# 924973292/EDITOR

Hardware: AMD Instinct MI355X
Metric: tri-modal images/sec fwd+bwd @ B=128 ViT-B (higher is better)
Workload: dtype bf16

## Files before the change

editor_amd/csrc/attention_bf16.hip:

```cpp
#include "common.h"
#include "../../include/editor_hip.h"
#include <type_traits>

#include "attn_common.h"
#include <string.h>

namespace {

#ifndef ATTN_ROLLOUT_SKIP
#define ATTN_ROLLOUT_SKIP 1
#endif
#ifndef ATTN_PAIR_SKIP
#define ATTN_PAIR_SKIP 0
#endif
#ifndef ATTN_UNROLL_BWD
#define ATTN_UNROLL_BWD 1
#endif

constexpr int STG_ROW = ROWB + 32, STG_BYTES = 16 * STG_ROW;
constexpr int STG_LPR = CPR <= 4 ? 4 : (CPR <= 8 ? 8 : 16);
template <bool F16>
__device__ __forceinline__ void store_tile(char* stg, const float4_t (&o)[ND], bf16_t* dst, long ldo, int nrows, int lane)
{
    const int li = lane & 15, lg = lane >> 4;
// ... 489 lines not shown
    if (kCols<NT> && a.colparts) {
        __syncthreads();
        float* red = reinterpret_cast<float*>(smem);
        wave_colsum_park(csk, red + (w * 2) * HD, lane);
        wave_colsum_park(csv, red + (w * 2 + 1) * HD, lane);
        __syncthreads();
        if (threadIdx.x < 2 * HD) {
            const int which = threadIdx.x / HD, c = threadIdx.x % HD;
            float t = 0.f;
            for (int i = 0; i < nw; ++i) t += red[(i * 2 + which) * HD + c];
            a.colparts[(long)b * 3 * D + (1 + which) * D + hh * HD + c] = t;
        }
    }
}

template <int NT, bool F16>
__global__ __launch_bounds__(256) __attribute__((amdgpu_waves_per_eu(4, 8))) void attn_rollout_step_kernel(const bf16_t* __restrict__ qkv, const float* __restrict__ lse,
    const float* __restrict__ r_in, int T, int heads, float scale, long Mtot, float* __restrict__ r_out, int final_step)
{
    extern __shared__ __attribute__((aligned(16))) char smem[];
    constexpr int Tp = NT * 16;
    char* qimg = smem;
    float* lse_s = reinterpret_cast<float*>(smem + Tp * ROWB);
    float* w_s = lse_s + Tp;
    const int D = heads * HD;
    const int b = blockIdx.x / heads, hh = blockIdx.x % heads;
    const long ld = 3L * D;
    const long row0 = (long)b * T;
    const int nt = min(NT, ((T + 31) >> 5) << 1);
    const int nu = !ATTN_ROLLOUT_SKIP ? nt : (r_in ? min(nt, (T + 15) >> 4) : 1);
// ... 7 lines not shown
    short8_t kn[KS];
#pragma unroll
    for (int s = 0; s < KS; ++s) kn[s] = frag_own(qbase + D, ld, w * 16, T, s, lane);
    images_ready();
    const int li = lane & 15, lg = lane >> 4;
    const float sc = scale * kLog2e;
    for (int k0 = w * 16; k0 < T; k0 += nw * 16) {
        const int key = k0 + li;
        short8_t kf[KS];
#pragma unroll
        for (int s = 0; s < KS; ++s) kf[s] = kn[s];
        if (k0 + nw * 16 < T) {
#pragma unroll
            for (int s = 0; s < KS; ++s) kn[s] = frag_own(qbase + D, ld, k0 + nw * 16, T, s, lane);
        }
        float acc = 0.f;
#pragma unroll 2
        for (int u = 0; u < nu; ++u) {
            float4_t s_ = {0.f, 0.f, 0.f, 0.f};
#pragma unroll
            for (int s = 0; s < KS; ++s)
                s_ = mfma16<F16>(frag_k(qimg, u * 16, s, lane), kf[s], s_);
            const float4 l4 = *reinterpret_cast<const float4*>(lse_s + 16 * u + 4 * lg);
            const float4 w4 = *reinterpret_cast<const float4*>(w_s + 16 * u + 4 * lg);
            acc = fmaf(__builtin_amdgcn_exp2f(s_[0] * sc - l4.x), w4.x, acc);
            acc = fmaf(__builtin_amdgcn_exp2f(s_[1] * sc - l4.y), w4.y, acc);
            acc = fmaf(__builtin_amdgcn_exp2f(s_[2] * sc - l4.z), w4.z, acc);
            acc = fmaf(__builtin_amdgcn_exp2f(s_[3] * sc - l4.w), w4.w, acc);
        }
        acc = group_sum(acc);
        if (lg == 0 && key < T) {
            if (final_step) { if (key >= 1) r_out[(long)blockIdx.x * (T - 1) + key - 1] = acc; }
            else r_out[(long)blockIdx.x * T + key] = acc;
        }
    }
}

constexpr int LCH = 256;

template <bool BWD, bool F16>
__global__ __launch_bounds__(256) __attribute__((amdgpu_waves_per_eu(4, 8))) void attn_q_long_kernel(AttnArgs a)
{
    extern __shared__ __attribute__((aligned(16))) char smem[];
    char* kimg = smem;
    char* vimg = smem + LCH * ROWB;
    const int D = a.heads * HD;
    const int b = blockIdx.x / a.heads, hh = blockIdx.x % a.heads;
    const long ld = 3L * D;
    const long row0 = a.cu ? (long)a.cu[b] : (long)b * a.T;
// ... 347 lines not shown
#define ROLL_CASE(NTV) case NTV: {                                                                                   \
        auto k = attn_rollout_step_kernel<NTV, F16>;                                                                     \
        const size_t lds = (size_t)NTV * 16 * ROWB + (size_t)2 * NTV * 16 * sizeof(float);                              \
        int rc = set_lds(k, lds); if (rc) return rc;                                                                     \
        hipLaunchKernelGGL(k, grid, dim3(threads), lds, stream, qkv, lse, r_in, T, heads, scale, Mtot, r_out, final_step); \
        break; }
    switch (pick_nt(T)) {
        ROLL_CASE(10) ROLL_CASE(14) ROLL_CASE(26) ROLL_CASE(38)
        default: return (int)hipErrorInvalidValue;
    }
#undef ROLL_CASE
    EDITOR_LAUNCH_CHECK();
    return 0;
}

}

#if ATTN_HD == 64
#define ATTN_ENTRY(name) name
#define ATTN_DECL_WIDTHS(name, ...) extern "C" int name##_hd32(__VA_ARGS__); extern "C" int name##_hd96(__VA_ARGS__);
#define ATTN_OTHER_WIDTHS(name, ...) do { if (hd == 32) return name##_hd32(__VA_ARGS__); if (hd == 96) return name##_hd96(__VA_ARGS__); } while (0)
#elif ATTN_HD == 32
#define ATTN_ENTRY(name) name##_hd32
#define ATTN_DECL_WIDTHS(name, ...)
#define ATTN_OTHER_WIDTHS(name, ...) do { } while (0)
#else
#define ATTN_ENTRY(name) name##_hd96
#define ATTN_DECL_WIDTHS(name, ...)
#define ATTN_OTHER_WIDTHS(name, ...) do { } while (0)
#endif
// ... 52 lines not shown
#define ROLL_ARGS const uint16_t* qkv, const float* lse, const float* r_in, int B, int T, int heads, int hd, float scale, \
                  float* r_out, int final_step, hipStream_t stream
ATTN_DECL_WIDTHS(editor_attn_rollout_step_bf16, ROLL_ARGS)
ATTN_DECL_WIDTHS(editor_attn_rollout_step_f16, ROLL_ARGS)
extern "C" int ATTN_ENTRY(editor_attn_rollout_step_bf16)(ROLL_ARGS)
{
    ATTN_OTHER_WIDTHS(editor_attn_rollout_step_bf16, qkv, lse, r_in, B, T, heads, hd, scale, r_out, final_step, stream);
    return rollout_step_h16<false>(qkv, lse, r_in, B, T, heads, hd, scale, r_out, final_step, stream);
}
extern "C" int ATTN_ENTRY(editor_attn_rollout_step_f16)(ROLL_ARGS)
{
    ATTN_OTHER_WIDTHS(editor_attn_rollout_step_f16, qkv, lse, r_in, B, T, heads, hd, scale, r_out, final_step, stream);
    return rollout_step_h16<true>(qkv, lse, r_in, B, T, heads, hd, scale, r_out, final_step, stream);
}
#undef ROLL_ARGS
```

editor_amd/csrc/gemm_f32.hip:

```cpp
#include "common.h"
#include "../../include/editor_hip.h"

typedef __attribute__((ext_vector_type(4))) float float4_t;

namespace {

constexpr int BM = 64, BN = 64, BK = 16, LDT = 80;

struct GemmArgs {
    const float* A; const float* B; float* C;
    int M, N, K;
    long lda, ldb, ldc;
    int transA, transB;
    int batch2; long sA1, sB1, sC1, sA2, sB2, sC2;
    float alpha, beta;
    const float* bias; const float* rowscale;
    int splitk;
    int epilogue; float* aux; long ldaux;
};

__device__ __forceinline__ float gelu_f(float a) { return 0.5f * a * (1.f + erff(a * 0.70710678118654752f)); }
__device__ __forceinline__ float gelu_grad_f(float a) {
    return 0.5f * (1.f + erff(a * 0.70710678118654752f)) + a * 0.3989422804014327f * __expf(-0.5f * a * a);
}

constexpr int NH = BK / 16;
struct TileRegs { float v[NH][4]; };

__device__ __forceinline__ void load_tile(const float* __restrict__ P, long ld, int trans, int r0, int k0, int R, int kend, TileRegs& t)
{
#pragma unroll
    for (int h = 0; h < NH; ++h) {
        const int c = threadIdx.x + 256 * h;
        float* v = t.v[h];
        v[0] = v[1] = v[2] = v[3] = 0.f;
        if (!trans) {
            const int r = c / (BK / 4), kk = (c % (BK / 4)) * 4;
            const int gr = r0 + r, gk = k0 + kk;
            if (gr < R) {
                const float* src = P + (long)gr * ld + gk;
                if (gk + 3 < kend && ((reinterpret_cast<uintptr_t>(src) & 15) == 0)) {
                    const float4 q = *reinterpret_cast<const float4*>(src);
                    v[0] = q.x; v[1] = q.y; v[2] = q.z; v[3] = q.w;
                } else {
#pragma unroll
                    for (int i = 0; i < 4; ++i) if (gk + i < kend) v[i] = src[i];
                }
            }
        } else {
            const int kk = c >> 4, r = (c & 15) * 4;
            const int gk = k0 + kk, gr = r0 + r;
            if (gk < kend) {
                const float* src = P + (long)gk * ld + gr;
                if (gr + 3 < R && ((reinterpret_cast<uintptr_t>(src) & 15) == 0)) {
                    const float4 q = *reinterpret_cast<const float4*>(src);
                    v[0] = q.x; v[1] = q.y; v[2] = q.z; v[3] = q.w;
                } else {
#pragma unroll
                    for (int i = 0; i < 4; ++i) if (gr + i < R) v[i] = src[i];
                }
            }
        }
    }
}
__device__ __forceinline__ void store_tile(const TileRegs& t, int trans, float (*S)[LDT])
{
#pragma unroll
    for (int h = 0; h < NH; ++h) {
        const int c = threadIdx.x + 256 * h;
        const float* v = t.v[h];
        if (!trans) {
            const int r = c / (BK / 4), kk = (c % (BK / 4)) * 4;
#pragma unroll
            for (int i = 0; i < 4; ++i) S[kk + i][r] = v[i];
        } else {
            const int kk = c >> 4, r = (c & 15) * 4;
            *reinterpret_cast<float4*>(&S[kk][r]) = make_float4(v[0], v[1], v[2], v[3]);
        }
    }
}

__global__ __launch_bounds__(256) __attribute__((amdgpu_waves_per_eu(4, 8))) void gemm_f32_kernel(GemmArgs g)
{
    __shared__ __attribute__((aligned(16))) float As[2][BK][LDT];
    __shared__ __attribute__((aligned(16))) float Bs[2][BK][LDT];
    const int z = blockIdx.z;
    const int split = z % g.splitk, bz = z / g.splitk;
    const int b1 = bz / g.batch2, b2 = bz % g.batch2;
    const float* A = g.A + b1 * g.sA1 + b2 * g.sA2;
    const float* B = g.B + b1 * g.sB1 + b2 * g.sB2;
    float* C = g.C + b1 * g.sC1 + b2 * g.sC2;
    const int m0 = blockIdx.y * BM, n0 = blockIdx.x * BN;
    const int ktiles = (g.K + BK - 1) / BK;
    const int per = (ktiles + g.splitk - 1) / g.splitk;
    const int kt0 = split * per, kt1 = min(ktiles, kt0 + per);
    const int lane = threadIdx.x & 63, w = threadIdx.x >> 6;
    const int wm = (w >> 1) * 32, wn = (w & 1) * 32;
    float4_t acc[2][2];
#pragma unroll
    for (int i = 0; i < 2; ++i)
#pragma unroll
        for (int j = 0; j < 2; ++j) acc[i][j] = float4_t{0.f, 0.f, 0.f, 0.f};

    TileRegs ra, rb;
    if (kt0 < kt1) {
        load_tile(A, g.lda, g.transA, m0, kt0 * BK, g.M, g.K, ra);
        load_tile(B, g.ldb, g.transB, n0, kt0 * BK, g.N, g.K, rb);
        store_tile(ra, g.transA, As[0]);
        store_tile(rb, g.transB, Bs[0]);
    }
    __syncthreads();
    for (int kt = kt0; kt < kt1; ++kt) {
        const int cur = (kt - kt0) & 1;
        const bool more = kt + 1 < kt1;
        if (more) {
            load_tile(A, g.lda, g.transA, m0, (kt + 1) * BK, g.M, g.K, ra);
            load_tile(B, g.ldb, g.transB, n0, (kt + 1) * BK, g.N, g.K, rb);
        }
#pragma unroll
        for (int ks = 0; ks < BK; ks += 4) {
            const int kr = ks + (lane >> 4);
            float a[2], b[2];
#pragma unroll
            for (int i = 0; i < 2; ++i) a[i] = As[cur][kr][wm + i * 16 + (lane & 15)];
#pragma unroll
            for (int j = 0; j < 2; ++j) b[j] = Bs[cur][kr][wn + j * 16 + (lane & 15)];
#pragma unroll
            for (int i = 0; i < 2; ++i)
#pragma unroll
                for (int j = 0; j < 2; ++j)
                    acc[i][j] = __builtin_amdgcn_mfma_f32_16x16x4f32(a[i], b[j], acc[i][j], 0, 0, 0);
        }
        if (more) {
            store_tile(ra, g.transA, As[cur ^ 1]);
            store_tile(rb, g.transB, Bs[cur ^ 1]);
        }
        __syncthreads();
    }
#pragma unroll
    for (int i = 0; i < 2; ++i)
#pragma unroll
        for (int j = 0; j < 2; ++j)
#pragma unroll
            for (int r = 0; r < 4; ++r) {
                const int m = m0 + wm + i * 16 + (lane >> 4) * 4 + r;
                const int n = n0 + wn + j * 16 + (lane & 15);
                if (m >= g.M || n >= g.N) continue;
                float v = g.alpha * acc[i][j][r];
                if (g.bias && split == 0) v += g.bias[n];
                if (g.rowscale) v *= g.rowscale[m];
                if (g.epilogue == EDITOR_EPI_RESIDUAL) v += g.aux[(long)m * g.ldaux + n];
                else if (g.epilogue == EDITOR_EPI_GELU) { g.aux[(long)m * g.ldaux + n] = v; v = gelu_f(v); }
                else if (g.epilogue == EDITOR_EPI_GELU_BWD) v *= gelu_grad_f(g.aux[(long)m * g.ldaux + n]);
                float* c = C + (long)m * g.ldc + n;
                if (g.splitk > 1) atomicAdd(c, v);
                else *c = g.beta != 0.f ? v + g.beta * *c : v;
            }
}

__global__ void scale_inplace_kernel(float* C, long rows, int cols, long ld, float beta)
{
    const long e = (long)blockIdx.x * blockDim.x + threadIdx.x;
    if (e >= rows * cols) return;
    float* c = C + (e / cols) * ld + (e % cols);
    *c = beta == 0.f ? 0.f : *c * beta;
}

}

extern "C" int editor_gemm_f32(const float* A, const float* B, float* C, int M, int N, int K, long lda, long ldb,
    long ldc, int transA, int transB, int batch1, long sA1, long sB1, long sC1, int batch2, long sA2, long sB2, long sC2,
    float alpha, float beta, const float* bias, const float* rowscale, int splitk, int epilogue, float* aux, long ldaux,
// ... 11 lines not shown
                float* c = C + b1 * sC1 + b2 * sC2;
                if (beta != 1.f) {
                    hipLaunchKernelGGL(scale_inplace_kernel, dim3((unsigned)(((long)M * N + 255) / 256)), dim3(256), 0,
                                       stream, c, (long)M, N, ldc, beta);
                    EDITOR_LAUNCH_CHECK();
                }
            }
    }
    GemmArgs g{A, B, C, M, N, K, lda, ldb, ldc, transA, transB, batch2, sA1, sB1, sC1, sA2, sB2, sC2,
               alpha, beta, bias, rowscale, splitk, epilogue, aux, ldaux};
    dim3 grid((N + BN - 1) / BN, (M + BM - 1) / BM, batch1 * batch2 * splitk);
    hipLaunchKernelGGL(gemm_f32_kernel, grid, dim3(256), 0, stream, g);
    EDITOR_LAUNCH_CHECK();
    return 0;
}
```

editor_amd/functional.py:

```python
import os
import weakref

import torch

from . import ops

_BF16_CACHE = {}
_WEIGHT_EPOCH = 0

F16_GRAD_SCALE = 32768.0


def set_f16_grad_scale(v):
    global F16_GRAD_SCALE
    v = float(v)
    if v <= 0 or (v != 2.0 ** round(__import__("math").log2(v))):
        raise ValueError("GRAD_SCALE must be a positive power of two")
    F16_GRAD_SCALE = v


def grad_scale(dtype):
    return F16_GRAD_SCALE if dtype == torch.float16 else 1.0


# ... 241 lines not shown



def _linear_bwd(*args, **kw):
    return _drive(_linear_bwd_gen(*args, **kw))


def _linear_bwd_gen(dy, x2d, w_act, need_bias, gelu_pre=None, m_live=None, db=None, dx_colsum=None, gs=1.0, dw_out=None,
                    db_out=None, dxcs_out=None, w_t=None, defer=None, aux_is_grad=True, rq=None, live_dense=False):
    m, n = dy.shape
    k = x2d.shape[1]
    inv = 1.0 / gs
    use_side = WGRAD_SIDE_STREAM and dy.dtype in ops.HALF_DTYPES and m >= 2048
    dy_ready = torch.cuda.current_stream(dy.device).record_event() if use_side else None
    dx = torch.empty(m, k, dtype=x2d.dtype, device=dy.device)
    dxcs = None
    if dx_colsum and ops.gemm_colsum_ok(m, k, n, dx.dtype, 0, 1, m_live, live_dense):
        dxcs = dxcs_out if dxcs_out is not None else torch.empty(k, dtype=torch.float32, device=dy.device)
    wb, ldb, tb = (w_t, n, 0) if w_t is not None else (w_act, k, 1)
    if gelu_pre is None:
        yield _GemmReq(dy, wb, dx, m, k, n, n, ldb, k, 0, tb, m_live=m_live, colsum=dxcs, colsum_scale=inv, tag="dgrad",
                       rq=rq, live_dense=live_dense)
    else:
        ag = ops.EPI_AUX_GRAD if (dy.dtype in ops.HALF_DTYPES and aux_is_grad) else 0
        yield _GemmReq(dy, wb, dx, m, k, n, n, ldb, k, 0, tb, epilogue=ops.EPI_GELU_BWD | ag | (STAGGER_FC2D if (m_live is None or live_dense) and m >= 16384 else 0),
                       aux=gelu_pre, m_live=m_live,
                       colsum=dxcs, colsum_scale=inv, tag="dgrad", rq=rq, live_dense=live_dense)
    dw = dw_out if dw_out is not None else torch.empty(n, k, dtype=torch.float32, device=dy.device)
    if need_bias and db is None:
        db = db_out if db_out is not None else torch.empty(n, dtype=torch.float32, device=dy.device)
# ... 619 lines not shown
```

editor_amd/ops.py:

```python
import ctypes
import os

import torch

from . import _lib

call = _lib.call
_raw_stream = _lib._raw_stream


def patch_grid(h, w, sy, sx=None):
    sx = sy if sx is None else sx
    return (h - 16) // sy + 1, (w - 16) // sx + 1


def freq_counts(rgb, nir, tir, m4=None, stride=16):
    b, c, h, w = rgb.shape
    if stride != 16:
        ny, nx = patch_grid(h, w, stride)
        counts = torch.empty(b, ny * nx, dtype=torch.int32, device=rgb.device)
        plane = torch.empty(b * h * (w // 16), dtype=torch.int16, device=rgb.device)
        if m4 is not None:
            call("editor_freq_counts_stride_nmod_f32", rgb.contiguous(), nir.contiguous(), tir.contiguous(), m4.contiguous(), 4,
                 b, c, h, w, int(stride), plane, counts)
# ... 23 lines not shown
    return mask


def frequency_mask(rgb, nir, tir, keep, m4=None, stride=16):
    counts = freq_counts(rgb, nir, tir, m4, stride)
    return topk_mask(counts, keep), counts


def attn_rollout(probs):
    l, b, h, t, ldp = probs.shape
    scores = torch.empty(b, h, t - 1, dtype=torch.float32, device=probs.device)
    call("editor_attn_rollout_f32", probs, l, b * h, t, ldp, b * h * t * ldp, scores)
    return scores


def attn_rollout_qk(layers, b, t, heads, hd, scale=None):
    dev = layers[0][0].device
    scores = torch.empty(b, heads, t - 1, dtype=torch.float32, device=dev)
    bufs = [torch.empty(b * heads, t, dtype=torch.float32, device=dev) for _ in range(2)]
    r_in = None
    for i, layer in enumerate(reversed(layers)):
        last = i == len(layers) - 1
        out = scores if last else bufs[i & 1]
        if len(layer) == 3:
            qkv, qkv_lo, lse = layer
            call("editor_attn_rollout_step_f16x2", qkv, qkv_lo, lse, r_in, b, t, heads, hd, float(scale or hd ** -0.5), out,
                 1 if last else 0)
        else:
            qkv, lse = layer
            call(_h16(qkv, "attn_rollout_step"), qkv, lse, r_in, b, t, heads, hd, float(scale or hd ** -0.5), out,
                 1 if last else 0)
        r_in = out
    return scores
# ... 6 lines not shown


_WS = {}
_WS_RETIRED = []


def workspace(device, nfloats):
    key = (device.type, device.index, _raw_stream(device.index if device.index is not None else torch.cuda.current_device()))
    ws = _WS.get(key)
    if ws is None or ws.numel() < nfloats:
        if ws is not None:
            _WS_RETIRED.append(ws)
        ws = torch.empty(max(int(nfloats), 1 << 22), dtype=torch.float32, device=device)
        _WS[key] = ws
    return ws


_ARENA = {}


class ReduceQueue:
    ARENA_FLOATS = 16 << 20

    def __init__(self, device, slot=0, nslots=1):
        key = (device.index, _raw_stream(device.index if device.index is not None else torch.cuda.current_device()))
        buf = _ARENA.get(key)
        if buf is None:
            buf = _ARENA[key] = torch.empty(self.ARENA_FLOATS, dtype=torch.float32, device=device)
        span = (self.ARENA_FLOATS // int(nslots)) // 64 * 64
        self.base, self.limit = int(slot) * span, (int(slot) + 1) * span
# ... 324 lines not shown

def gemm_tile_plan(m, n, cus=256):
    th = gemm_tile_rows(m, n, cus)
    tiles_pp = -(-m // th) * ((n + 255) // 256)
    tiles_pipe = -(-m // 256) * ((n + 127) // 128)
    cost_pp = -(-tiles_pp // cus) * (0.95 if th == 208 else 1.0)
    cost_pipe = -(-tiles_pipe // cus) * 0.69
    return th, cost_pipe < 0.97 * cost_pp


def gemm_colsum_ok(m, n, k, c_dtype, trans_a, splitk, m_live, live_dense=False):
    return (c_dtype in HALF_DTYPES and not trans_a and splitk == 1 and (m_live is None or live_dense) and m >= 2048 and n >= 512
            and n % 8 == 0 and k % 64 == 0)


def gemm(a, b, c, m, n, k, lda, ldb, ldc, trans_a=0, trans_b=0, alpha=1.0, beta=0.0, bias=None, rowscale=None,
         splitk=1, a_off=0, b_off=0, c_off=0, epilogue=0, aux=None, m_live=None, colsum=None, colsum_scale=1.0, tag=None,
         rq=None, live_dense=False, rowmap=None):
    if a.dtype == torch.float32:
        assert b.dtype == torch.float32 and c.dtype == torch.float32 and m_live is None
        if (splitk == 1 and not trans_a and not trans_b and m <= 512 and k >= 1024 and k % 128 == 0 and epilogue == 0
                and rowscale is None and beta == 0.0 and ldc == n and a_off == b_off == c_off == 0):
            s_ = 8
            kc = k // s_
            slabs = workspace(a.device, (s_ - 1) * m * n)
            call("editor_gemm_f32", a, b, c, m, n, kc, lda, ldb, ldc, 0, 0, 1, 0, 0, 0, 1, 0, 0, 0, float(alpha), 0.0, bias,
                 None, 1, 0, None, n)
            call("editor_gemm_f32", _ptr(a, kc), _ptr(b, kc), slabs, m, n, kc, lda, ldb, n, 0, 0, s_ - 1, kc, kc, m * n,
                 1, 0, 0, 0, float(alpha), 0.0, None, None, 1, 0, None, n)
            call("editor_reduce_rows", slabs, s_ - 1, m * n, c, 1, 1.0)
            return
        call("editor_gemm_f32", _ptr(a, a_off), _ptr(b, b_off), _ptr(c, c_off), m, n, k, lda, ldb, ldc,
             int(trans_a), int(trans_b), 1, 0, 0, 0, 1, 0, 0, 0, float(alpha), float(beta), bias, rowscale, int(splitk),
             int(epilogue) & 0xFF, aux, n)
    elif a.dtype in HALF_DTYPES:
        assert b.dtype == a.dtype
        entry = _h16(a, "gemm")
        if m_live is not None and (m < 256 or n < 128 or k % 64):
            raise RuntimeError("live-row GEMM needs the pipelined path (M >= 256, N >= 128, K % 64 == 0)")
# ... 538 lines not shown
```

include/editor_hip.h:

```cpp
#ifndef EDITOR_HIP_H
#define EDITOR_HIP_H
#include <stdint.h>
#ifdef __cplusplus
extern "C" {
#endif

typedef struct ihipStream_t* editor_stream_t;

#define EDITOR_EPI_NONE 0
#define EDITOR_EPI_RESIDUAL 1
#define EDITOR_EPI_GELU 2
#define EDITOR_EPI_GELU_BWD 3
#define EDITOR_EPI_COLSUM 0x100
#define EDITOR_EPI_AUX_GRAD 0x400
#define EDITOR_EPI_FORCE_PP 0x200
#define EDITOR_EPI_PIPE128 0x800
#define EDITOR_EPI_STAGGER(c) (((c) & 63) << 17)
#define EDITOR_EPI_TILE_ROWS(h) ((((h) / 16) & 15) << 12)


int editor_freq_counts_f32(const float* rgb, const float* nir, const float* tir, int B, int C, int H, int W,
                           int32_t* counts, editor_stream_t stream);

int editor_freq_counts_nmod_f32(const float* m0, const float* m1, const float* m2, const float* m3, int nmod, int B, int C,
// ... 83 lines not shown

int editor_sfts_apply(const float* feat, const uint8_t* index, int nmod, long B, int T, int D, float* out,
                      float* loss, float* workspace, int ws_len, editor_stream_t stream);
int editor_sfts_apply_bwd(const float* feat, const uint8_t* index, const float* dout, const float* dloss, int nmod,
                          long B, int T, int D, float* dfeat, editor_stream_t stream);
int editor_pool_fwd(const float* x, long B, int nmod, int T, int D, float* out, float* num, editor_stream_t stream);
int editor_pool_bwd(const float* dout, const float* num, long B, int nmod, int T, int D, float* dx,
                    editor_stream_t stream);
int editor_rowmask_mul(float* x, const uint8_t* rowmask, int period, long M, int D, editor_stream_t stream);


int editor_gemm_f32(const float* A, const float* B, float* C, int M, int N, int K, long lda, long ldb, long ldc,
                    int transA, int transB, int batch1, long sA1, long sB1, long sC1, int batch2, long sA2, long sB2,
                    long sC2, float alpha, float beta, const float* bias, const float* rowscale, int splitk,
                    int epilogue, float* aux, long ldaux, editor_stream_t stream);

int editor_gemm_bf16(const uint16_t* A, const uint16_t* B, void* C, int c_f32, int M, int N, int K, long lda, long ldb,
                     long ldc, int transA, int transB, float alpha, float beta, const float* bias,
                     const float* rowscale, int splitk, int epilogue, void* aux, long ldaux,
                     float* splitk_ws ,
                     const int* m_live , editor_stream_t stream);

int editor_gemm_f16x2(const uint16_t* A_hi, const uint16_t* A_lo, const uint16_t* B_hi, const uint16_t* B_lo, void* C,
                      void* C_lo, int c_f32, int M, int N, int K, long lda, long ldb, long ldc, float alpha,
                      const float* bias, const float* rowscale, int epilogue, void* aux, long ldaux, const int* m_live,
                      editor_stream_t stream);

int editor_gemm_wgrad_group(int dtype, int count, const uint16_t* const* dy, const uint16_t* const* x, float* const* dw,
                            const int* N, const int* K, int M, float alpha, int splitk, float* ws, const int* m_live,
                            editor_stream_t stream);
// ... 12 lines not shown
int editor_gemm_f16(const uint16_t* A, const uint16_t* B, void* C, int c_f32, int M, int N, int K, long lda, long ldb,
                    long ldc, int transA, int transB, float alpha, float beta, const float* bias,
                    const float* rowscale, int splitk, int epilogue, void* aux, long ldaux, float* splitk_ws,
                    const int* m_live, editor_stream_t stream);


int editor_attention_fwd_f32(const float* qkv, int B, int T, int heads, int hd, float scale, const uint8_t* mask,
                             float* out, float* probs, editor_stream_t stream);
int editor_attention_bwd_f32(const float* qkv, const float* dout, const float* probs, int B, int T, int heads, int hd,
                             float scale, float* dqkv, float* workspace, editor_stream_t stream);

int editor_attn_rollout_step_bf16(const uint16_t* qkv, const float* lse, const float* r_in, int B, int T, int heads, int hd,
                                  float scale, float* r_out, int final_step, editor_stream_t stream);
int editor_attn_rollout_step_f16(const uint16_t* qkv, const float* lse, const float* r_in, int B, int T, int heads, int hd,
                                 float scale, float* r_out, int final_step, editor_stream_t stream);

int editor_attention_fwd_bf16(const uint16_t* qkv, int B, int T, int heads, int hd, float scale, const uint8_t* mask,
                              uint16_t* out, float* probs, int ldp , float* lse,
                              const int* cu, long Mtot, editor_stream_t stream);
int editor_attention_bwd_bf16(const uint16_t* qkv, const uint16_t* dout, const uint16_t* out, const float* lse, int B,
                              int T, int heads, int hd, float scale, const uint8_t* mask, uint16_t* dqkv,
                              float* workspace, const int* cu, long Mtot, editor_stream_t stream);
int editor_attention_bwd_colsum_bf16(const uint16_t* qkv, const uint16_t* dout, const uint16_t* out, const float* lse, int B,
                                     int T, int heads, int hd, float scale, const uint8_t* mask, uint16_t* dqkv,
                                     float* workspace, const int* cu, long Mtot, float* colparts, editor_stream_t stream);
int editor_attention_bwd_colsum_f16(const uint16_t* qkv, const uint16_t* dout, const uint16_t* out, const float* lse, int B,
                                    int T, int heads, int hd, float scale, const uint8_t* mask, uint16_t* dqkv,
                                    float* workspace, const int* cu, long Mtot, float* colparts, editor_stream_t stream);
int editor_attention_fwd_f16x2(const uint16_t* qkv_hi, const uint16_t* qkv_lo, int B, int T, int heads, int hd, float scale,
                               const uint8_t* mask, uint16_t* out_hi, uint16_t* out_lo, float* probs, int ldp, float* lse,
// ... 136 lines not shown
```

Measured before the change: 3138.

## Add single-launch attention rollout, fused f32 linear backward and chunked split-K GEMM

Adds a persistent rollout kernel that walks all layers inside one launch, double-buffering Q images, keys and LSE in LDS and registers, but it sits behind an environment flag that is off by default. It also restructures the f32 GEMM tile layout into an MFMA-fragment-friendly LDS image and factors out the main loop. A new one-launch f32 linear backward computes dx, dw and db together, and a chunked split-K kernel uses tickets for in-kernel reduction; both are enabled by default. The aim is to cut kernel-launch counts and separate reduction passes on the small f32 linears, at the cost of extra workspace and ticket state.

Result: no change. 3161 (median of 6 runs) (+0.8%).

```diff
diff --git a/editor_amd/csrc/attention_bf16.hip b/editor_amd/csrc/attention_bf16.hip
--- a/editor_amd/csrc/attention_bf16.hip
+++ b/editor_amd/csrc/attention_bf16.hip
@@ -527,6 +527,28 @@
     }
 }
 
+template <bool F16>
+__device__ __forceinline__ float rollout_key_tile(const char* qimg, const float* lse_s, const float* w_s, const short8_t (&kf)[KS],
+                                                  int nu, float sc, int lane)
+{
+    const int lg = lane >> 4;
+    float acc = 0.f;
+#pragma unroll 2
+    for (int u = 0; u < nu; ++u) {
+        float4_t s_ = {0.f, 0.f, 0.f, 0.f};
+#pragma unroll
+        for (int s = 0; s < KS; ++s)
+            s_ = mfma16<F16>(frag_k(qimg, u * 16, s, lane), kf[s], s_);
+        const float4 l4 = *reinterpret_cast<const float4*>(lse_s + 16 * u + 4 * lg);
+        const float4 w4 = *reinterpret_cast<const float4*>(w_s + 16 * u + 4 * lg);
+        acc = fmaf(__builtin_amdgcn_exp2f(s_[0] * sc - l4.x), w4.x, acc);
+        acc = fmaf(__builtin_amdgcn_exp2f(s_[1] * sc - l4.y), w4.y, acc);
+        acc = fmaf(__builtin_amdgcn_exp2f(s_[2] * sc - l4.z), w4.z, acc);
+        acc = fmaf(__builtin_amdgcn_exp2f(s_[3] * sc - l4.w), w4.w, acc);
+    }
+    return group_sum(acc);
+}
+
 template <int NT, bool F16>
 __global__ __launch_bounds__(256) __attribute__((amdgpu_waves_per_eu(4, 8))) void attn_rollout_step_kernel(const bf16_t* __restrict__ qkv, const float* __restrict__ lse,
     const float* __restrict__ r_in, int T, int heads, float scale, long Mtot, float* __restrict__ r_out, int final_step)
@@ -564,25 +586,105 @@
 #pragma unroll
             for (int s = 0; s < KS; ++s) kn[s] = frag_own(qbase + D, ld, k0 + nw * 16, T, s, lane);
         }
-        float acc = 0.f;
-#pragma unroll 2
-        for (int u = 0; u < nu; ++u) {
-            float4_t s_ = {0.f, 0.f, 0.f, 0.f};
-#pragma unroll
-            for (int s = 0; s < KS; ++s)
-                s_ = mfma16<F16>(frag_k(qimg, u * 16, s, lane), kf[s], s_);
-            const float4 l4 = *reinterpret_cast<const float4*>(lse_s + 16 * u + 4 * lg);
-            const float4 w4 = *reinterpret_cast<const float4*>(w_s + 16 * u + 4 * lg);
-            acc = fmaf(__builtin_amdgcn_exp2f(s_[0] * sc - l4.x), w4.x, acc);
-            acc = fmaf(__builtin_amdgcn_exp2f(s_[1] * sc - l4.y), w4.y, acc);
-            acc = fmaf(__builtin_amdgcn_exp2f(s_[2] * sc - l4.z), w4.z, acc);
-            acc = fmaf(__builtin_amdgcn_exp2f(s_[3] * sc - l4.w), w4.w, acc);
-        }
-        acc = group_sum(acc);
+        const float acc = rollout_key_tile<F16>(qimg, lse_s, w_s, kf, nu, sc, lane);
         if (lg == 0 && key < T) {
             if (final_step) { if (key >= 1) r_out[(long)blockIdx.x * (T - 1) + key - 1] = acc; }
             else r_out[(long)blockIdx.x * T + key] = acc;
         }
+    }
+}
+
+constexpr int ROLL_MAXL = 32;
+struct RolloutLayers { const bf16_t* qkv[ROLL_MAXL]; const float* lse[ROLL_MAXL]; };
+
+template <int NT> constexpr int kRollTiles = NT <= 10 ? 3 : 4;
+
+template <int NT, bool F16>
+__global__ __launch_bounds__(256) __attribute__((amdgpu_waves_per_eu(3, 8))) void attn_rollout_kernel(RolloutLayers tab, int L, int T, int heads,
+    float scale, long Mtot, float* __restrict__ scores)
+{
+    extern __shared__ __attribute__((aligned(16))) char smem[];
+    constexpr int Tp = NT * 16;
+    constexpr int LPT = (Tp + 191) / 192;
+    constexpr int MT = kRollTiles<NT>;
+    float* lse_s = reinterpret_cast<float*>(smem + 2 * Tp * ROWB);
+    float* w_s = lse_s + 2 * Tp;
+    const int D = heads * HD;
+    const int b = blockIdx.x / heads, hh = blockIdx.x % heads;
+    const long ld = 3L * D;
+    const long row0 = (long)b * T;
+    const long hoff = row0 * ld + hh * HD;
+    const long loff = (long)hh * Mtot + row0;
+    const int nt = min(NT, ((T + 31) >> 5) << 1);
+    const int nfull = !ATTN_ROLLOUT_SKIP ? nt : min(nt, (T + 15) >> 4);
+    const int lane = threadIdx.x & 63, w = threadIdx.x >> 6, nw = blockDim.x >> 6;
+    const int li = lane & 15, lg = lane >> 4;
+    const float sc = scale * kLog2e;
+    float lse_r[LPT];
+    auto request_keys = [&](short8_t (&k)[MT][KS], const bf16_t* kbase) {
+#pragma unroll
+        for (int j = 0; j < MT; ++j) {
+            const int k0 = (w + j * nw) * 16;
+            if (k0 < T) {
+#pragma unroll
+                for (int s = 0; s < KS; ++s) k[j][s] = frag_own(kbase, ld, k0, T, s, lane);
+            }
+        }
+    };
+    auto request_lse = [&](const float* src) {
+#pragma unroll
+        for (int j = 0; j < LPT; ++j) {
+            const int t = threadIdx.x + j * blockDim.x;
+            lse_r[j] = t < T ? src[loff + t] : INFINITY;
+        }
+    };
+    auto layer = [&](int i, const short8_t (&kc)[MT][KS], short8_t (&kx)[MT][KS]) {
+        const int l = L - 1 - i, cur = i & 1, nxt = cur ^ 1;
+        const bool more = l > 0;
+        images_ready();
+        const char* qimg = smem + cur * Tp * ROWB;
+        const float* lse_c = lse_s + cur * Tp;
+        const float* w_c = w_s + cur * Tp;
+        float* w_n = w_s + nxt * Tp;
+        if (more) {
+            const bf16_t* nbase = tab.qkv[l - 1] + hoff;
+            request_keys(kx, nbase + D);
+            request_lse(tab.lse[l - 1]);
+            load_image(smem + nxt * Tp * ROWB, nbase, ld, T, nt * 16);
+        }
+        const int nu = !ATTN_ROLLOUT_SKIP ? nt : (i ? nfull : 1);
+#pragma unroll
+        for (int j = 0; j < MT; ++j) {
+            const int k0 = (w + j * nw) * 16;
+            if (k0 < T) {
+                const int key = k0 + li;
+                const float acc = rollout_key_tile<F16>(qimg, lse_c, w_c, kc[j], nu, sc, lane);
+                if (lg == 0 && key < T) {
+                    if (more) w_n[key] = acc;
+                    else if (key >= 1) scores[(long)blockIdx.x * (T - 1) + key - 1] = acc;
+                }
+            }
+        }
+        if (more) {
+#pragma unroll
+            for (int j = 0; j < LPT; ++j) {
+                const int t = threadIdx.x + j * blockDim.x;
+                if (t < Tp) lse_s[nxt * Tp + t] = lse_r[j];
+            }
+        }
+    };
+    short8_t ka[MT][KS], kb[MT][KS];
+    request_keys(ka, tab.qkv[L - 1] + hoff + D);
+    request_lse(tab.lse[L - 1]);
+    load_image(smem, tab.qkv[L - 1] + hoff, ld, T, (ATTN_ROLLOUT_SKIP ? 1 : nt) * 16);
+#pragma unroll
+    for (int j = 0; j < LPT; ++j) {
+        const int t = threadIdx.x + j * blockDim.x;
+        if (t < Tp) { lse_s[t] = lse_r[j]; w_s[t] = t == 0 ? 1.f : 0.f; w_s[Tp + t] = 0.f; }
+    }
+    for (int i = 0; i < L; i += 2) {
+        layer(i, ka, kb);
+        if (i + 1 < L) layer(i + 1, kb, ka);
     }
 }
 
@@ -960,6 +1062,35 @@
     return 0;
 }
 
+template <bool F16>
+int rollout_h16(int L, const uint16_t* const* qkv, const float* const* lse, int B, int T, int heads, int hd, float scale,
+                float* scores, hipStream_t stream)
+{
+    if (hd != HD || T < 2 || B < 1 || L < 1 || L > ROLL_MAXL || !qkv || !lse || !scores) return (int)hipErrorInvalidValue;
+    RolloutLayers tab;
+    for (int l = 0; l < ROLL_MAXL; ++l) {
+        tab.qkv[l] = qkv[l < L ? l : 0]; tab.lse[l] = lse[l < L ? l : 0];
+        if (!tab.qkv[l] || !tab.lse[l]) return (int)hipErrorInvalidValue;
+    }
+    const int threads = pick_threads(T);
+    const dim3 grid(B * heads);
+    const long Mtot = (long)B * T;
+#define ROLL_CASE(NTV) case NTV: {                                                                                   \
+        if (((T + 15) / 16 + threads / 64 - 1) / (threads / 64) > kRollTiles<NTV>) return (int)hipErrorInvalidValue;     \
+        auto k = attn_rollout_kernel<NTV, F16>;                                                                          \
+        const size_t lds = (size_t)2 * NTV * 16 * ROWB + (size_t)4 * NTV * 16 * sizeof(float);                          \
+        int rc = set_lds(k, lds); if (rc) return rc;                                                                     \
+        hipLaunchKernelGGL(k, grid, dim3(threads), lds, stream, tab, L, T, heads, scale, Mtot, scores);                  \
+        break; }
+    switch (pick_nt(T)) {
+        ROLL_CASE(10) ROLL_CASE(14)
+        default: return (int)hipErrorInvalidValue;
+    }
+#undef ROLL_CASE
+    EDITOR_LAUNCH_CHECK();
+    return 0;
+}
+
 }
 
 #if ATTN_HD == 64
@@ -1042,3 +1173,19 @@
     return rollout_step_h16<true>(qkv, lse, r_in, B, T, heads, hd, scale, r_out, final_step, stream);
 }
 #undef ROLL_ARGS
+
+#define ROLLALL_ARGS int L, const uint16_t* const* qkv, const float* const* lse, int B, int T, int heads, int hd, float scale, \
+                     float* scores, hipStream_t stream
+ATTN_DECL_WIDTHS(editor_attn_rollout_bf16, ROLLALL_ARGS)
+ATTN_DECL_WIDTHS(editor_attn_rollout_f16, ROLLALL_ARGS)
+extern "C" int ATTN_ENTRY(editor_attn_rollout_bf16)(ROLLALL_ARGS)
+{
+    ATTN_OTHER_WIDTHS(editor_attn_rollout_bf16, L, qkv, lse, B, T, heads, hd, scale, scores, stream);
+    return rollout_h16<false>(L, qkv, lse, B, T, heads, hd, scale, scores, stream);
+}
+extern "C" int ATTN_ENTRY(editor_attn_rollout_f16)(ROLLALL_ARGS)
+{
+    ATTN_OTHER_WIDTHS(editor_attn_rollout_f16, L, qkv, lse, B, T, heads, hd, scale, scores, stream);
+    return rollout_h16<true>(L, qkv, lse, B, T, heads, hd, scale, scores, stream);
+}
+#undef ROLLALL_ARGS
diff --git a/editor_amd/csrc/gemm_f32.hip b/editor_amd/csrc/gemm_f32.hip
--- a/editor_amd/csrc/gemm_f32.hip
+++ b/editor_amd/csrc/gemm_f32.hip
@@ -5,7 +5,8 @@
 
 namespace {
 
-constexpr int BM = 64, BN = 64, BK = 16, LDT = 80;
+constexpr int BM = 64, BN = 64, BK = 16;
+constexpr int TILE_F = 64 * BK;
 
 struct GemmArgs {
     const float* A; const float* B; float* C;
@@ -24,66 +25,92 @@
     return 0.5f * (1.f + erff(a * 0.70710678118654752f)) + a * 0.3989422804014327f * __expf(-0.5f * a * a);
 }
 
-constexpr int NH = BK / 16;
-struct TileRegs { float v[NH][4]; };
+static_assert(BK == 16, "the tile image is written for BK = 16");
+struct TileRegs { float v[4]; };
 
 __device__ __forceinline__ void load_tile(const float* __restrict__ P, long ld, int trans, int r0, int k0, int R, int kend, TileRegs& t)
 {
-#pragma unroll
-    for (int h = 0; h < NH; ++h) {
-        const int c = threadIdx.x + 256 * h;
-        float* v = t.v[h];
-        v[0] = v[1] = v[2] = v[3] = 0.f;
-        if (!trans) {
-            const int r = c / (BK / 4), kk = (c % (BK / 4)) * 4;
-            const int gr = r0 + r, gk = k0 + kk;
-            if (gr < R) {
-                const float* src = P + (long)gr * ld + gk;
-                if (gk + 3 < kend && ((reinterpret_cast<uintptr_t>(src) & 15) == 0)) {
-                    const float4 q = *reinterpret_cast<const float4*>(src);
-                    v[0] = q.x; v[1] = q.y; v[2] = q.z; v[3] = q.w;
-                } else {
-#pragma unroll
-                    for (int i = 0; i < 4; ++i) if (gk + i < kend) v[i] = src[i];
-                }
+    const int c = threadIdx.x;
+    float* v = t.v;
+    v[0] = v[1] = v[2] = v[3] = 0.f;
+    if (!trans) {
+        const int r = c / (BK / 4), kk = (c % (BK / 4)) * 4;
+        const int gr = r0 + r, gk = k0 + kk;
+        if (gr < R) {
+            const float* src = P + (long)gr * ld + gk;
+            if (gk + 3 < kend && ((reinterpret_cast<uintptr_t>(src) & 15) == 0)) {
+                const float4 q = *reinterpret_cast<const float4*>(src);
+                v[0] = q.x; v[1] = q.y; v[2] = q.z; v[3] = q.w;
+            } else {
+#pragma unroll
+                for (int i = 0; i < 4; ++i) if (gk + i < kend) v[i] = src[i];
             }
-        } else {
-            const int kk = c >> 4, r = (c & 15) * 4;
-            const int gk = k0 + kk, gr = r0 + r;
-            if (gk < kend) {
-                const float* src = P + (long)gk * ld + gr;
-                if (gr + 3 < R && ((reinterpret_cast<uintptr_t>(src) & 15) == 0)) {
-                    const float4 q = *reinterpret_cast<const float4*>(src);
-                    v[0] = q.x; v[1] = q.y; v[2] = q.z; v[3] = q.w;
-                } else {
-#pragma unroll
-                    for (int i = 0; i < 4; ++i) if (gr + i < R) v[i] = src[i];
-                }
-            }
-        }
-    }
-}
-__device__ __forceinline__ void store_tile(const TileRegs& t, int trans, float (*S)[LDT])
-{
-#pragma unroll
-    for (int h = 0; h < NH; ++h) {
-        const int c = threadIdx.x + 256 * h;
-        const float* v = t.v[h];
-        if (!trans) {
-            const int r = c / (BK / 4), kk = (c % (BK / 4)) * 4;
-#pragma unroll
-            for (int i = 0; i < 4; ++i) S[kk + i][r] = v[i];
-        } else {
-            const int kk = c >> 4, r = (c & 15) * 4;
-            *reinterpret_cast<float4*>(&S[kk][r]) = make_float4(v[0], v[1], v[2], v[3]);
-        }
+        }
+    } else {
+        const int gr = r0 + (c & 63), gk = k0 + (c >> 6);
+        if (gr < R) {
+#pragma unroll
+            for (int j = 0; j < 4; ++j) if (gk + 4 * j < kend) v[j] = P[(long)(gk + 4 * j) * ld + gr];
+        }
+    }
+}
+__device__ __forceinline__ void store_tile(const TileRegs& t, int trans, float* S)
+{
+    const int c = threadIdx.x;
+    const float* v = t.v;
+    if (!trans) {
+#pragma unroll
+        for (int i = 0; i < 4; ++i) S[i * 256 + c] = v[i];
+    } else {
+        *reinterpret_cast<float4*>(S + (c >> 6) * 256 + (c & 63) * 4) = make_float4(v[0], v[1], v[2], v[3]);
+    }
+}
+
+__device__ __forceinline__ void gemm_mainloop(const float* __restrict__ A, const float* __restrict__ B, long lda, long ldb, int transA,
+    int transB, int m0, int n0, int M, int N, int K, int kt0, int kt1, float* As, float* Bs, float4_t (&acc)[2][2])
+{
+    const int lane = threadIdx.x & 63, w = threadIdx.x >> 6;
+    const int wm = (w >> 1) * 32, wn = (w & 1) * 32;
+    const int fa = (lane >> 4) * 256 + (wm + (lane & 15)) * 4, fb = (lane >> 4) * 256 + (wn + (lane & 15)) * 4;
+    TileRegs ra, rb;
+    if (kt0 < kt1) {
+        load_tile(A, lda, transA, m0, kt0 * BK, M, K, ra);
+        load_tile(B, ldb, transB, n0, kt0 * BK, N, K, rb);
+        store_tile(ra, transA, As);
+        store_tile(rb, transB, Bs);
+    }
+    __syncthreads();
+    for (int kt = kt0; kt < kt1; ++kt) {
+        const int cur = (kt - kt0) & 1;
+        const bool more = kt + 1 < kt1;
+        if (more) {
+            load_tile(A, lda, transA, m0, (kt + 1) * BK, M, K, ra);
+            load_tile(B, ldb, transB, n0, (kt + 1) * BK, N, K, rb);
+        }
+        float4_t a[2], b[2];
+#pragma unroll
+        for (int i = 0; i < 2; ++i) a[i] = *reinterpret_cast<const float4_t*>(As + cur * TILE_F + fa + i * 64);
+#pragma unroll
+        for (int j = 0; j < 2; ++j) b[j] = *reinterpret_cast<const float4_t*>(Bs + cur * TILE_F + fb + j * 64);
+#pragma unroll
+        for (int ks = 0; ks < BK / 4; ++ks)
+#pragma unroll
+            for (int i = 0; i < 2; ++i)
+#pragma unroll
+                for (int j = 0; j < 2; ++j)
+                    acc[i][j] = __builtin_amdgcn_mfma_f32_16x16x4f32(a[i][ks], b[j][ks], acc[i][j], 0, 0, 0);
+        if (more) {
+            store_tile(ra, transA, As + (cur ^ 1) * TILE_F);
+            store_tile(rb, transB, Bs + (cur ^ 1) * TILE_F);
+        }
+        __syncthreads();
     }
 }
 
 __global__ __launch_bounds__(256) __attribute__((amdgpu_waves_per_eu(4, 8))) void gemm_f32_kernel(GemmArgs g)
 {
-    __shared__ __attribute__((aligned(16))) float As[2][BK][LDT];
-    __shared__ __attribute__((aligned(16))) float Bs[2][BK][LDT];
+    __shared__ __attribute__((aligned(16))) float As[2 * TILE_F];
+    __shared__ __attribute__((aligned(16))) float Bs[2 * TILE_F];
     const int z = blockIdx.z;
     const int split = z % g.splitk, bz = z / g.splitk;
     const int b1 = bz / g.batch2, b2 = bz % g.batch2;
@@ -101,42 +128,7 @@
     for (int i = 0; i < 2; ++i)
 #pragma unroll
         for (int j = 0; j < 2; ++j) acc[i][j] = float4_t{0.f, 0.f, 0.f, 0.f};
-
-    TileRegs ra, rb;
-    if (kt0 < kt1) {
-        load_tile(A, g.lda, g.transA, m0, kt0 * BK, g.M, g.K, ra);
-        load_tile(B, g.ldb, g.transB, n0, kt0 * BK, g.N, g.K, rb);
-        store_tile(ra, g.transA, As[0]);
-        store_tile(rb, g.transB, Bs[0]);
-    }
-    __syncthreads();
-    for (int kt = kt0; kt < kt1; ++kt) {
-        const int cur = (kt - kt0) & 1;
-        const bool more = kt + 1 < kt1;
-        if (more) {
-            load_tile(A, g.lda, g.transA, m0, (kt + 1) * BK, g.M, g.K, ra);
-            load_tile(B, g.ldb, g.transB, n0, (kt + 1) * BK, g.N, g.K, rb);
-        }
-#pragma unroll
-        for (int ks = 0; ks < BK; ks += 4) {
-            const int kr = ks + (lane >> 4);
-            float a[2], b[2];
-#pragma unroll
-            for (int i = 0; i < 2; ++i) a[i] = As[cur][kr][wm + i * 16 + (lane & 15)];
-#pragma unroll
-            for (int j = 0; j < 2; ++j) b[j] = Bs[cur][kr][wn + j * 16 + (lane & 15)];
-#pragma unroll
-            for (int i = 0; i < 2; ++i)
-#pragma unroll
-                for (int j = 0; j < 2; ++j)
-                    acc[i][j] = __builtin_amdgcn_mfma_f32_16x16x4f32(a[i], b[j], acc[i][j], 0, 0, 0);
-        }
-        if (more) {
-            store_tile(ra, g.transA, As[cur ^ 1]);
-            store_tile(rb, g.transB, Bs[cur ^ 1]);
-        }
-        __syncthreads();
-    }
+    gemm_mainloop(A, B, g.lda, g.ldb, g.transA, g.transB, m0, n0, g.M, g.N, g.K, kt0, kt1, As, Bs, acc);
 #pragma unroll
     for (int i = 0; i < 2; ++i)
 #pragma unroll
@@ -156,6 +148,141 @@
                 if (g.splitk > 1) atomicAdd(c, v);
                 else *c = g.beta != 0.f ? v + g.beta * *c : v;
             }
+}
+
+constexpr int kChunks = 8;
+struct ChunkedArgs {
+    const float* A; const float* B; float* C; float* slabs; unsigned* tickets;
+    int M, N, K; long lda, ldb;
+    float alpha; const float* bias;
+};
+
+__global__ __launch_bounds__(256) __attribute__((amdgpu_waves_per_eu(4, 8))) void linear_f32_chunked_kernel(ChunkedArgs g)
+{
+    __shared__ __attribute__((aligned(16))) float smem[4 * TILE_F];
+    float* As = smem;
+    float* Bs = smem + 2 * TILE_F;
+    const int chunk = blockIdx.z;
+    const int kc = g.K / kChunks;
+    const int m0 = blockIdx.y * BM, n0 = blockIdx.x * BN;
+    const int lane = threadIdx.x & 63, w = threadIdx.x >> 6;
+    const int wm = (w >> 1) * 32, wn = (w & 1) * 32;
+    float4_t acc[2][2];
+#pragma unroll
+    for (int i = 0; i < 2; ++i)
+#pragma unroll
+        for (int j = 0; j < 2; ++j) acc[i][j] = float4_t{0.f, 0.f, 0.f, 0.f};
+    gemm_mainloop(g.A + (long)chunk * kc, g.B + (long)chunk * kc, g.lda, g.ldb, 0, 0, m0, n0, g.M, g.N, kc, 0, kc / BK, As, Bs, acc);
+    const long MN = (long)g.M * g.N;
+    float* slab = g.slabs + chunk * MN;
+#pragma unroll
+    for (int i = 0; i < 2; ++i)
+#pragma unroll
+        for (int j = 0; j < 2; ++j)
+#pragma unroll
+            for (int r = 0; r < 4; ++r) {
+                const int m = m0 + wm + i * 16 + (lane >> 4) * 4 + r;
+                const int n = n0 + wn + j * 16 + (lane & 15);
+                if (m >= g.M || n >= g.N) continue;
+                float v = g.alpha * acc[i][j][r];
+                if (g.bias && chunk == 0) v += g.bias[n];
+                slab[(long)m * g.N + n] = v;
+            }
+    asm volatile("s_waitcnt vmcnt(0)" ::: "memory");
+    __syncthreads();
+    unsigned* flag = reinterpret_cast<unsigned*>(smem);
+    if (threadIdx.x == 0) {
+        __builtin_amdgcn_fence(__ATOMIC_RELEASE, "agent");
+        asm volatile("s_waitcnt vmcnt(0)" ::: "memory");
+        unsigned* cnt = g.tickets + blockIdx.y * gridDim.x + blockIdx.x;
+        const unsigned t = __hip_atomic_fetch_add(cnt, 1u, __ATOMIC_RELAXED, __HIP_MEMORY_SCOPE_AGENT);
+        const bool last = t == (unsigned)(kChunks - 1);
+        if (last) {
+            __hip_atomic_store(cnt, 0u, __ATOMIC_RELAXED, __HIP_MEMORY_SCOPE_AGENT);
+            __builtin_amdgcn_fence(__ATOMIC_ACQUIRE, "agent");
+            asm volatile("s_waitcnt vmcnt(0)" ::: "memory");
+        }
+        *flag = last ? 1u : 0u;
+    }
+    __syncthreads();
+    if (!*flag) return;
+    const float* sl = g.slabs;
+    const int cols = min(BN, g.N - n0), rows = min(BM, g.M - m0);
+#pragma unroll 4
+    for (int e = threadIdx.x; e < BM * BN; e += 256) {
+        const int r = e >> 6, c = e & 63;
+        if (r >= rows || c >= cols) continue;
+        const long idx = (long)(m0 + r) * g.N + n0 + c;
+        float p[kChunks];
+#pragma unroll
+        for (int q = 0; q < kChunks; ++q) p[q] = sl[q * MN + idx];
+        float t = 0.f;
+#pragma unroll
+        for (int q = 1; q < kChunks; ++q) t += p[q];
+        g.C[idx] = p[0] + t;
+    }
+}
+
+struct LinearBwdArgs {
+    const float* dy; const float* x; const float* w;
+    float* dx; float* dw; float* db;
+    int M, N, K;
+    float alpha_w, db_scale;
+    int dx_tiles, dw_tiles;
+};
+
+__global__ __launch_bounds__(256) __attribute__((amdgpu_waves_per_eu(4, 8))) void linear_f32_bwd_kernel(LinearBwdArgs g)
+{
+    __shared__ __attribute__((aligned(16))) float smem[4 * TILE_F];
+    int bid = blockIdx.x;
+    const int lane = threadIdx.x & 63, w = threadIdx.x >> 6;
+    if (bid < g.dx_tiles + g.dw_tiles) {
+        const bool wgrad = bid >= g.dx_tiles;
+        if (wgrad) bid -= g.dx_tiles;
+        const int tiles_x = (g.K + BN - 1) / BN;
+        const int m0 = (bid / tiles_x) * BM, n0 = (bid % tiles_x) * BN;
+        const int Mp = wgrad ? g.N : g.M, Kp = wgrad ? g.M : g.N;
+        const float alpha = wgrad ? g.alpha_w : 1.f;
+        float* C = wgrad ? g.dw : g.dx;
+        const int wm = (w >> 1) * 32, wn = (w & 1) * 32;
+        float4_t acc[2][2];
+#pragma unroll
+        for (int i = 0; i < 2; ++i)
+#pragma unroll
+            for (int j = 0; j < 2; ++j) acc[i][j] = float4_t{0.f, 0.f, 0.f, 0.f};
+        gemm_mainloop(g.dy, wgrad ? g.x : g.w, g.N, g.K, wgrad ? 1 : 0, 1, m0, n0, Mp, g.K, Kp, 0, (Kp + BK - 1) / BK, smem,
+                      smem + 2 * TILE_F, acc);
+#pragma unroll
+        for (int i = 0; i < 2; ++i)
+#pragma unroll
+            for (int j = 0; j < 2; ++j)
+#pragma unroll
+                for (int r = 0; r < 4; ++r) {
+                    const int m = m0 + wm + i * 16 + (lane >> 4) * 4 + r;
+                    const int n = n0 + wn + j * 16 + (lane & 15);
+                    if (m >= Mp || n >= g.K) continue;
+                    C[(long)m * g.K + n] = alpha * acc[i][j][r];
+                }
+        return;
+    }
+    bid -= g.dx_tiles + g.dw_tiles;
+    float (*red)[64] = reinterpret_cast<float (*)[64]>(smem);
+    const int c = bid * 64 + lane, rg = w;
+    float t = 0.f;
+    for (int r0 = 0; r0 < g.M; r0 += 64) {
+        const int r1 = min(g.M, r0 + 64);
+        float a = 0.f, b = 0.f;
+        if (c < g.N) {
+            int r = r0 + rg;
+            for (; r + 4 < r1; r += 8) { a += g.dy[(long)r * g.N + c]; b += g.dy[(long)(r + 4) * g.N + c]; }
+            if (r < r1) a += g.dy[(long)r * g.N + c];
+        }
+        red[rg][lane] = a + b;
+        __syncthreads();
+        if (rg == 0) t += 0.f + ((red[0][lane] + red[1][lane]) + (red[2][lane] + red[3][lane]));
+        __syncthreads();
+    }
+    if (rg == 0 && c < g.N) g.db[c] = t * g.db_scale;
 }
 
 __global__ void scale_inplace_kernel(float* C, long rows, int cols, long ld, float beta)
@@ -197,3 +324,26 @@
     EDITOR_LAUNCH_CHECK();
     return 0;
 }
+
+extern "C" int editor_linear_f32_chunked(const float* A, const float* B, float* C, int M, int N, int K, long lda, long ldb,
+    float alpha, const float* bias, float* slabs, unsigned* tickets, hipStream_t stream)
+{
+    if (M <= 0 || N <= 0 || K <= 0 || K % (kChunks * BK) || !A || !B || !C || !slabs || !tickets) return (int)hipErrorInvalidValue;
+    ChunkedArgs g{A, B, C, slabs, tickets, M, N, K, lda, ldb, alpha, bias};
+    dim3 grid((N + BN - 1) / BN, (M + BM - 1) / BM, kChunks);
+    hipLaunchKernelGGL(linear_f32_chunked_kernel, grid, dim3(256), 0, stream, g);
+    EDITOR_LAUNCH_CHECK();
+    return 0;
+}
+
+extern "C" int editor_linear_f32_bwd(const float* dy, const float* x, const float* w, int M, int N, int K, float alpha_w, float* dx,
+    float* dw, float* db, float db_scale, hipStream_t stream)
+{
+    if (M <= 0 || N <= 0 || K <= 0 || M > 1024 || !dy || !x || !w || !dx || !dw || (db && N % 4)) return (int)hipErrorInvalidValue;
+    const int tiles_x = (K + BN - 1) / BN;
+    LinearBwdArgs g{dy, x, w, dx, dw, db, M, N, K, alpha_w, db_scale, ((M + BM - 1) / BM) * tiles_x, ((N + BM - 1) / BM) * tiles_x};
+    const int blocks = g.dx_tiles + g.dw_tiles + (db ? (N + 63) / 64 : 0);
+    hipLaunchKernelGGL(linear_f32_bwd_kernel, dim3(blocks), dim3(256), 0, stream, g);
+    EDITOR_LAUNCH_CHECK();
+    return 0;
+}
diff --git a/editor_amd/functional.py b/editor_amd/functional.py
--- a/editor_amd/functional.py
+++ b/editor_amd/functional.py
@@ -279,6 +279,15 @@
     use_side = WGRAD_SIDE_STREAM and dy.dtype in ops.HALF_DTYPES and m >= 2048
     dy_ready = torch.cuda.current_stream(dy.device).record_event() if use_side else None
     dx = torch.empty(m, k, dtype=x2d.dtype, device=dy.device)
+    if (gelu_pre is None and m_live is None and db is None and not dx_colsum and w_t is None and defer is None
+            and ops.linear_f32_bwd_ok(dy, x2d, w_act, need_bias)):
+        dw = dw_out if dw_out is not None else torch.empty(n, k, dtype=torch.float32, device=dy.device)
+        if need_bias:
+            db = db_out if db_out is not None else torch.empty(n, dtype=torch.float32, device=dy.device)
+        ops.linear_f32_bwd(dy, x2d, w_act, dx, dw, db if need_bias else None, inv)
+        if dx_colsum is not None:
+            return dx, dw, (db if need_bias else None), None
+        return dx, dw, (db if need_bias else None)
     dxcs = None
     if dx_colsum and ops.gemm_colsum_ok(m, k, n, dx.dtype, 0, 1, m_live, live_dense):
         dxcs = dxcs_out if dxcs_out is not None else torch.empty(k, dtype=torch.float32, device=dy.device)
diff --git a/editor_amd/ops.py b/editor_amd/ops.py
--- a/editor_amd/ops.py
+++ b/editor_amd/ops.py
@@ -61,9 +61,22 @@
     return scores
 
 
+ROLLOUT_ONE_LAUNCH = os.environ.get("EDITOR_ROLLOUT_ONE_LAUNCH", "0") == "1"
+
+
 def attn_rollout_qk(layers, b, t, heads, hd, scale=None):
     dev = layers[0][0].device
     scores = torch.empty(b, heads, t - 1, dtype=torch.float32, device=dev)
+    if (ROLLOUT_ONE_LAUNCH and t <= 224 and len(layers) <= 32 and all(len(layer) == 2 for layer in layers)
+            and len({layer[0].dtype for layer in layers}) == 1):
+        n = len(layers)
+        qkvs = (ctypes.c_void_p * n)(*[layer[0].data_ptr() for layer in layers])
+        lses = (ctypes.c_void_p * n)(*[layer[1].data_ptr() for layer in layers])
+        for qkv, lse in layers:
+            if not (qkv.is_cuda and qkv.is_contiguous() and lse.is_cuda and lse.is_contiguous()):
+                raise RuntimeError("attn_rollout_qk: layer tensors must be contiguous GPU tensors")
+        call(_h16(layers[0][0], "attn_rollout"), n, qkvs, lses, b, t, heads, hd, float(scale or hd ** -0.5), scores)
+        return scores
     bufs = [torch.empty(b * heads, t, dtype=torch.float32, device=dev) for _ in range(2)]
     r_in = None
     for i, layer in enumerate(reversed(layers)):
@@ -100,6 +113,20 @@
         ws = torch.empty(max(int(nfloats), 1 << 22), dtype=torch.float32, device=device)
         _WS[key] = ws
     return ws
+
+
+_TICKETS = {}
+_TICKETS_RETIRED = []
+
+
+def tickets(device, n):
+    key = (device.type, device.index, _raw_stream(device.index if device.index is not None else torch.cuda.current_device()))
+    t = _TICKETS.get(key)
+    if t is None or t.numel() < n:
+        if t is not None:
+            _TICKETS_RETIRED.append(t)
+        t = _TICKETS[key] = torch.zeros(max(int(n), 4096), dtype=torch.int32, device=device)
+    return t
 
 
 _ARENA = {}
@@ -454,6 +481,19 @@
             and n % 8 == 0 and k % 64 == 0)
 
 
+LINEAR_ONE_LAUNCH = os.environ.get("EDITOR_LINEAR_ONE_LAUNCH", "1") != "0"
+
+
+def linear_f32_bwd_ok(dy, x, w, need_bias):
+    return (LINEAR_ONE_LAUNCH and dy.dtype == x.dtype == w.dtype == torch.float32 and dy.shape[0] <= 512
+            and not (need_bias and dy.shape[1] % 4))
+
+
+def linear_f32_bwd(dy, x, w, dx, dw, db=None, scale=1.0):
+    m, n = dy.shape
+    call("editor_linear_f32_bwd", dy, x, w, m, n, x.shape[1], float(scale), dx, dw, db, float(scale))
+
+
 def gemm(a, b, c, m, n, k, lda, ldb, ldc, trans_a=0, trans_b=0, alpha=1.0, beta=0.0, bias=None, rowscale=None,
          splitk=1, a_off=0, b_off=0, c_off=0, epilogue=0, aux=None, m_live=None, colsum=None, colsum_scale=1.0, tag=None,
          rq=None, live_dense=False, rowmap=None):
@@ -463,6 +503,11 @@
                 and rowscale is None and beta == 0.0 and ldc == n and a_off == b_off == c_off == 0):
             s_ = 8
             kc = k // s_
+            if LINEAR_ONE_LAUNCH and lda == k and ldb == k:
+                slabs = workspace(a.device, s_ * m * n)
+                call("editor_linear_f32_chunked", a, b, c, m, n, k, lda, ldb, float(alpha), bias, slabs,
+                     tickets(a.device, -(-m // 64) * -(-n // 64)))
+                return
             slabs = workspace(a.device, (s_ - 1) * m * n)
             call("editor_gemm_f32", a, b, c, m, n, kc, lda, ldb, ldc, 0, 0, 1, 0, 0, 0, 1, 0, 0, 0, float(alpha), 0.0, bias,
                  None, 1, 0, None, n)
diff --git a/include/editor_hip.h b/include/editor_hip.h
--- a/include/editor_hip.h
+++ b/include/editor_hip.h
@@ -121,6 +121,10 @@
                     int transA, int transB, int batch1, long sA1, long sB1, long sC1, int batch2, long sA2, long sB2,
                     long sC2, float alpha, float beta, const float* bias, const float* rowscale, int splitk,
                     int epilogue, float* aux, long ldaux, editor_stream_t stream);
+int editor_linear_f32_bwd(const float* dy, const float* x, const float* w, int M, int N, int K, float alpha_w, float* dx,
+                          float* dw, float* db, float db_scale, editor_stream_t stream);
+int editor_linear_f32_chunked(const float* A, const float* B, float* C, int M, int N, int K, long lda, long ldb, float alpha,
+                              const float* bias, float* slabs, unsigned* tickets, editor_stream_t stream);
 
 int editor_gemm_bf16(const uint16_t* A, const uint16_t* B, void* C, int c_f32, int M, int N, int K, long lda, long ldb,
                      long ldc, int transA, int transB, float alpha, float beta, const float* bias,
@@ -163,6 +167,10 @@
                                   float scale, float* r_out, int final_step, editor_stream_t stream);
 int editor_attn_rollout_step_f16(const uint16_t* qkv, const float* lse, const float* r_in, int B, int T, int heads, int hd,
                                  float scale, float* r_out, int final_step, editor_stream_t stream);
+int editor_attn_rollout_bf16(int L, const uint16_t* const* qkv, const float* const* lse, int B, int T, int heads, int hd,
+                             float scale, float* scores, editor_stream_t stream);
+int editor_attn_rollout_f16(int L, const uint16_t* const* qkv, const float* const* lse, int B, int T, int heads, int hd,
+                            float scale, float* scores, editor_stream_t stream);
 
 int editor_attention_fwd_bf16(const uint16_t* qkv, int B, int T, int heads, int hd, float scale, const uint8_t* mask,
                               uint16_t* out, float* probs, int ldp , float* lse,
```
